# utiasDSL/safe-control-gym

Hardware: AMD Instinct MI355X
Metric: env-steps/sec (whole node), Quadrotor2D-track (higher is better)
Workload: dtype f32; 1 GPU; quadrotor_2D_track: 65536 envs/GPU x 1 GPU, 1 launch of the fused step kernel per control step (20 engine substeps, obs/reward/done/info/constraints, auto-reset), synthetic U(-1,1) actions resident in HBM, HIP graph of 82 steps; envs_per_gpu=65536, task_yaml=safe_control_gym_amd/configs/quadrotor_2D_track.yaml, parallelism=env-shard x1, rccl_ranks=1, kernel_build=config-specialised, timing=one timed region of 82 steps

## Files before the change

### include/scg_learn.h

```cpp
#ifndef SCG_LEARN_H
#define SCG_LEARN_H

#include <stddef.h>
#include <stdint.h>

#ifdef __cplusplus
extern "C" {
#endif

typedef struct {
    int32_t W1, b1;
    int32_t W2, b2;
    int32_t W3, b3;
} scg_mlp_layout;

void scg_learn_shape(int32_t* obs_dim, int32_t* hidden, int32_t* act_dim, int32_t* activation);

int scg_mlp_forward(const float* d_params, const scg_mlp_layout* layout, int nout, const float* d_x, int m, float* d_out,
                    const uint8_t* d_row_mask, void* stream);

typedef struct {
    const float* d_params;
    scg_mlp_layout actor, critic;
    int32_t logstd_off;
    int32_t n_params;
    const float* d_obs;
    const float* d_act;
    const float* d_logp_old;
    const float* d_adv;
    const float* d_ret;
    const float* d_v_old;
    const int32_t* d_idx;
    int32_t batch;
    float clip_param, entropy_coef;
    int32_t use_clipped_value;
    int32_t n_workgroups;
    void* d_workspace;
    float* d_grad;
    float* d_stats;
} scg_ppo_grad_args;
size_t scg_ppo_grad_workspace_bytes(int n_workgroups);
int scg_ppo_grad(const scg_ppo_grad_args* args, void* stream);

int scg_adam_gated(float* d_p, const float* d_g, float* d_m, float* d_v, int n, int n_actor, float lr_actor, float lr_critic,
                   float* d_steps, float target_kl, float* d_stats_acc, const float* d_stats, uint32_t* d_block_counter,
                   void* stream);
int scg_adam_gated_scaled(float* d_p, const float* d_g, float* d_m, float* d_v, int n, int n_actor, float lr_actor, float lr_critic,
                          float* d_steps, float target_kl, float* d_stats_acc, const float* d_stats, uint32_t* d_block_counter,
                          float grad_scale, void* stream);

int scg_ppo_step(const scg_ppo_grad_args* args, float* d_m, float* d_v, float lr_actor, float lr_critic, const float* d_steps_in,
                 float* d_steps_out, float target_kl, float* d_stats_acc, void* stream);

void scg_learn_force_accumulating_form(int on);

int scg_ppo_returns_prepare(const uint8_t* d_done, const uint8_t* d_flags, const float* d_rew, const float* d_v_all, int T, int N,
                            uint8_t* d_trunc, float* d_mask, float* d_rew_out, float* d_v_out, void* stream);
size_t scg_ppo_returns_scratch_bytes(void);
int scg_ppo_returns_moments(const float* d_adv, int T, int N, float* d_episode_acc, void* d_scratch, double* d_moments,
                            float* d_episode_totals, void* stream);
int scg_ppo_returns_normalise(const float* d_adv, const double* d_moments, int T, int N, float* d_out, void* stream);

int scg_random_permutation(int32_t* d_out, int n, int count, uint64_t key, void* stream);
int scg_random_permutation_keyed(int32_t* d_out, int n, int count, const uint64_t* d_key_state, uint32_t epoch_offset, void* stream);

const char* scg_learn_last_error(void);
const char* scg_learn_source_hash_tag(void);

#ifdef __cplusplus
}
#endif
#endif
```

### safe_control_gym_amd/_learn.py

```python
import ctypes as C
import os

from safe_control_gym_amd import _lib as L
from safe_control_gym_amd import _shapelib

ACTS = {'tanh': 0, 'relu': 1, 'leaky_relu': 2}
SRC = os.path.join(L.CSRC_DIR, 'scg_learn.hip')
DEPS = [SRC, os.path.join(L.CSRC_DIR, 'scg_adam.h'), os.path.join(L.CSRC_DIR, 'scg_mlp.h'), os.path.join(L.CSRC_DIR, 'scg_once.h'), os.path.normpath(os.path.join(L.CSRC_DIR, '..', '..', 'include', 'scg_learn.h'))]


class MlpLayout(C.Structure):
    _fields_ = [(n, C.c_int32) for n in ('W1', 'b1', 'W2', 'b2', 'W3', 'b3')]


class PpoGradArgs(C.Structure):
    _fields_ = [('d_params', C.c_void_p), ('actor', MlpLayout), ('critic', MlpLayout), ('logstd_off', C.c_int32),
                ('n_params', C.c_int32), ('d_obs', C.c_void_p), ('d_act', C.c_void_p), ('d_logp_old', C.c_void_p),
                ('d_adv', C.c_void_p), ('d_ret', C.c_void_p), ('d_v_old', C.c_void_p), ('d_idx', C.c_void_p),
                ('batch', C.c_int32), ('clip_param', C.c_float), ('entropy_coef', C.c_float),
                ('use_clipped_value', C.c_int32), ('n_workgroups', C.c_int32), ('d_workspace', C.c_void_p),
                ('d_grad', C.c_void_p), ('d_stats', C.c_void_p)]


def supported(obs_dim, hidden, act_dim, activation):
    return (1 <= obs_dim <= 31 and hidden % 32 == 0 and 32 <= hidden <= 128 and act_dim in (1, 2, 4) and activation in ACTS)


def source_hash():
    return _shapelib.source_hash(DEPS)


def lib_path(obs_dim, hidden, act_dim, activation):
    tag = os.environ.get('SCG_LEARN_TAG', '')
    return os.path.join(L.SPEC_DIR, f'libscg_learn_{obs_dim}_{hidden}_{act_dim}_{activation}{"_" + tag if tag else ""}.so')


def build(obs_dim, hidden, act_dim, activation, force=False):
    if not supported(obs_dim, hidden, act_dim, activation):
        raise L.ScgError(f'no MFMA learner for obs {obs_dim} hidden {hidden} act {act_dim} {activation}')
    defines = {'SCG_L_NIN': obs_dim, 'SCG_L_H': hidden, 'SCG_L_NU': act_dim, 'SCG_L_ACT': ACTS[activation]}
    return _shapelib.build(lib_path(obs_dim, hidden, act_dim, activation), SRC, DEPS, defines, 'learner', 'SCG_LEARN_FLAGS', force)
# ... 36 lines not shown
```

### safe_control_gym_amd/csrc/scg_learn.hip

```cpp
#include <hip/hip_runtime.h>

#include <algorithm>
#include <cstdint>
#include <cstdio>
#include <cstdlib>
#include <string>

#include "../../include/scg_learn.h"
#include "scg_adam.h"
#include "scg_mlp.h"
#include "scg_once.h"

#ifndef SCG_L_NIN
#error "compile with -DSCG_L_NIN= -DSCG_L_H= -DSCG_L_NU= -DSCG_L_ACT="
#endif

using namespace scg;

#ifndef SCG_L_PART_AUX
#define SCG_L_PART_AUX 17
#endif
constexpr int NIN = SCG_L_NIN, HID = SCG_L_H, NU = SCG_L_NU, ACT = SCG_L_ACT;
constexpr int NT = HID / 32;
constexpr int XS_WORDS = (NIN + 2) * 32;
constexpr int WAVES = 4;

static thread_local std::string g_err;
static int fail(int code, const std::string& m) { g_err = m; return code; }
extern "C" const char* scg_learn_last_error(void) { return g_err.c_str(); }
extern "C" void scg_learn_shape(int32_t* nin, int32_t* hidden, int32_t* nu, int32_t* act) {
    *nin = NIN; *hidden = HID; *nu = NU; *act = ACT;
}
#ifndef SCG_SRC_HASH
#define SCG_SRC_HASH 0ULL
#endif
#define SCG_STR2(x) #x
#define SCG_STR(x) SCG_STR2(x)
extern "C" const char* scg_learn_source_hash_tag(void) { return "SCG_SRC_HASH:" SCG_STR(SCG_SRC_HASH); }

#define HIP_TRY(e) do { hipError_t _e = (e); if (_e != hipSuccess) return fail(-2, std::string(#e) + ": " + hipGetErrorString(_e)); } while (0)

__host__ __device__ static inline MlpWeights weights_of(const float* p, const scg_mlp_layout& L) {
    return MlpWeights{p + L.W1, p + L.b1, p + L.W2, p + L.b2, p + L.W3, p + L.b3};
}

template <int L1Q>
__device__ __forceinline__ void load_x(const float* __restrict__ obs, int sample, int h, float* x) {
#pragma unroll
    for (int g = 0; g < L1Q / 4; ++g) {
        const int r0 = 8 * g + 4 * h;
        if constexpr (NIN % 4 == 0) {
            f32x4 v = {0.0f, 0.0f, 0.0f, 0.0f};
            if (r0 < NIN) v = *reinterpret_cast<const f32x4*>(obs + (size_t)sample * NIN + r0);
            x[4 * g + 0] = v.x; x[4 * g + 1] = v.y; x[4 * g + 2] = v.z; x[4 * g + 3] = v.w;
        } else {
#pragma unroll
            for (int r = 0; r < 4; ++r) x[4 * g + r] = (r0 + r < NIN) ? obs[(size_t)sample * NIN + r0 + r] : 0.0f;
        }
    }
}

#ifndef SCG_L_FWD_WAVES
#define SCG_L_FWD_WAVES 8
#endif
constexpr int FWD_WAVES = SCG_L_FWD_WAVES;
constexpr int FWD_FILL = FWD_WAVES > 8 ? 512 : 64 * FWD_WAVES;
template <int NOUT>
__global__ __launch_bounds__(64 * FWD_WAVES) void mlp_forward_kernel(const float* __restrict__ params, const scg_mlp_layout lay,
                                                          const float* __restrict__ xin, int M, float* __restrict__ out,
                                                          const uint8_t* __restrict__ row_mask) {
    using L = MlpLds<NIN, HID, NOUT>;
    extern __shared__ __align__(16) float lds[];
    const MlpWeights w = weights_of(params, lay);
    if (FWD_FILL == 64 * FWD_WAVES || (int)threadIdx.x < FWD_FILL) mlp_fill_lds<NIN, HID, NOUT, 20, FWD_FILL>(lds, w, threadIdx.x);
    __syncthreads();
    const int lane = threadIdx.x & 63, wave = threadIdx.x >> 6;
    const int c = lane & 31, h = lane >> 5;
    const int n_tiles = (M + 31) / 32;
    for (int tile = blockIdx.x * (blockDim.x >> 6) + wave; tile < n_tiles; tile += gridDim.x * (blockDim.x >> 6)) {
        int s = tile * 32 + c;
        const bool live = s < M;
        s = live ? s : M - 1;
        if (row_mask) {
            const bool want = live && row_mask[s] != 0;
            if (__ballot(want) == 0ull) {
                if (live && h == 0) {
#pragma unroll
                    for (int k = 0; k < NOUT; ++k) out[(size_t)s * NOUT + k] = 0.0f;
                }
                continue;
            }
        }
        float x[L::L1Q];
        load_x<L::L1Q>(xin, s, h, x);
        f32x16 h1[NT], h2[NT];
        float o[NOUT];
        mlp_forward_tile<NIN, HID, NOUT, ACT>(lds, x, h1, h2, o, lane);
        if (live && h == 0) {
            const bool keep = !row_mask || row_mask[s] != 0;
#pragma unroll
            for (int k = 0; k < NOUT; ++k) out[(size_t)s * NOUT + k] = keep ? o[k] : 0.0f;
        }
    }
}

template <int NOUT>
struct GradLds {
    static constexpr int DW1 = 0;
    static constexpr int DB1 = DW1 + NIN * HID;
    static constexpr int DB2 = DB1 + HID;
    static constexpr int DW3 = DB2 + HID;
    static constexpr int DB3 = DW3 + NOUT * HID;
    static constexpr int DLS = DB3 + 4;
    static constexpr int STAT = DLS + 4;
    static constexpr int END = STAT + 4;
};
template <int NOUT> constexpr int partial_small() { return GradLds<NOUT>::END; }
template <int NOUT> constexpr int partial_words() { return GradLds<NOUT>::END + HID * HID; }
constexpr int PARTIAL_STRIDE = partial_words<(NU > 1 ? NU : 1)>();

constexpr int W1R = GradLds<(NU > 1 ? NU : 1)>::END;
constexpr size_t grad_lds_base_words() {
    size_t a = MlpLds<NIN, HID, NU>::END + GradLds<NU>::END;
    size_t c = MlpLds<NIN, HID, 1>::END + GradLds<1>::END;
    return (a > c ? a : c) + WAVES * XS_WORDS + WAVES * 4 * 32 + WAVES * TR_WORDS;
}
constexpr bool private_dw1() { return (grad_lds_base_words() + (WAVES - 1) * W1R) * sizeof(float) <= 160 * 1024; }
constexpr int PUB_TILE = 1024;
constexpr size_t scratch_words() { return WAVES * XS_WORDS + WAVES * 4 * 32 + WAVES * TR_WORDS + (private_dw1() ? (WAVES - 1) * W1R : 0); }
template <int NOUT>
constexpr size_t region_b_words() {
    constexpr size_t in_image = MlpLds<NIN, HID, NOUT>::END / PUB_TILE, need = 2 * WAVES * (HID / 32);
    constexpr size_t rest = need > in_image ? (need - in_image) * PUB_TILE : 0;
    return rest > scratch_words() ? rest : scratch_words();
}
static_assert(NIN < 32, "the dW1 product appends a column of ones: NIN + 1 <= 32");

struct GradArgs {
    const float* params; scg_mlp_layout actor, critic; int logstd_off;
    const float* obs; const float* act; const float* logp_old; const float* adv; const float* ret; const float* v_old;
    const int32_t* idx; int batch;
    float clip_param; int use_clipped_value;
    float* partials;
};

#ifdef SCG_L_TIMING
#define SCG_L_SLOTS reinterpret_cast<unsigned long long*>(A.partials + (size_t)gridDim.x * 2 * PARTIAL_STRIDE)
#define SCG_L_STAMP(k) do { if (ACTOR && blockIdx.x == 0 && threadIdx.x == 0) SCG_L_SLOTS[k] = __builtin_readcyclecounter(); } while (0)
#define SCG_L_TSTAMP(k) do { tst[k] = __builtin_readcyclecounter(); } while (0)
#else
#define SCG_L_STAMP(k) do {} while (0)
#define SCG_L_TSTAMP(k) do {} while (0)
#endif

__device__ __forceinline__ void gl_add(float* p, float v) {
    if constexpr (private_dw1()) *p += v;
    else atomicAdd(p, v);
}

template <int NOUT, bool ACTOR, bool ONE>
__device__ __forceinline__ void grad_net(const GradArgs& A, float* lds) {
    using L = MlpLds<NIN, HID, NOUT>;
    using G = GradLds<NOUT>;
    constexpr int L1Q = L::L1Q;
    float* const gl = lds + L::END;
    float* const xs_all = gl + G::END;
    float* const dout_all = xs_all + WAVES * XS_WORDS;
    float* const scr_all = dout_all + WAVES * 4 * 32;
    float* const w1_all = scr_all + WAVES * TR_WORDS;
    const int tid = threadIdx.x, lane = tid & 63, wave = tid >> 6;
    const int c = lane & 31, h = lane >> 5;
    const MlpWeights w = weights_of(A.params, ACTOR ? A.actor : A.critic);
    SCG_L_STAMP(0);
    const int n_tiles = A.batch / 32;
    const int tile0 = blockIdx.x * WAVES + wave;
    const int s_pre = A.idx[tile0 < n_tiles ? tile0 * 32 + c : c];
    float x_pre[L1Q], act_pre[NOUT], a_pre = 0.0f, b_pre = 0.0f;
    if constexpr (ONE) {
        mlp_fill_lds<NIN, HID, NOUT>(lds, w, tid, [&]() {
            load_x<L1Q>(A.obs, s_pre, h, x_pre);
            if constexpr (ACTOR) {
#pragma unroll
                for (int a = 0; a < NOUT; ++a) act_pre[a] = A.act[(size_t)s_pre * NOUT + a];
                a_pre = A.logp_old[s_pre]; b_pre = A.adv[s_pre];
            } else {
                a_pre = A.ret[s_pre];
                if (A.use_clipped_value) b_pre = A.v_old[s_pre];
            }
        });
    } else {
        mlp_fill_lds<NIN, HID, NOUT>(lds, w, tid);
    }
    for (int k = tid; k < G::END; k += blockDim.x) gl[k] = 0.0f;
    if constexpr (private_dw1()) {
// ... 37 lines not shown
#ifdef SCG_L_TIMING
        unsigned long long tst[10];
#endif
        SCG_L_TSTAMP(0);
        float x[L1Q];
        float s_act[NOUT], s_a = 0.0f, s_b = 0.0f;
        if constexpr (ONE) {
#pragma unroll
            for (int q = 0; q < L1Q; ++q) x[q] = x_pre[q];
#pragma unroll
            for (int a = 0; a < NOUT; ++a) s_act[a] = act_pre[a];
            s_a = a_pre; s_b = b_pre;
        } else {
            const int s = tile == tile0 ? s_pre : A.idx[tile * 32 + c];
            load_x<L1Q>(A.obs, s, h, x);
            if constexpr (ACTOR) {
#pragma unroll
                for (int a = 0; a < NOUT; ++a) s_act[a] = A.act[(size_t)s * NOUT + a];
                s_a = A.logp_old[s]; s_b = A.adv[s];
            } else {
                s_a = A.ret[s];
                if (A.use_clipped_value) s_b = A.v_old[s];
            }
        }
#pragma unroll
        for (int q = 0; q < L1Q; ++q) {
            const int f = d_row(q, 0);
            if (f + 4 < NIN) xs[(f + 4 * h) * 32 + c] = x[q];
            else if (f < NIN) { if (h == 0) xs[f * 32 + c] = x[q]; }
        }
        SCG_L_TSTAMP(1);
        float out[NOUT], dout[NOUT];
#ifdef SCG_L_TIMING
        mlp_forward_tile<NIN, HID, NOUT, ACT, 20, ACT, ONE>(lds, x, h1, h2, out, lane, tst + 8);
#else
        mlp_forward_tile<NIN, HID, NOUT, ACT, 20, ACT, ONE>(lds, x, h1, h2, out, lane);
#endif
        SCG_L_TSTAMP(2);
        if constexpr (ACTOR) {
            float logp = 0.0f, z[NOUT];
#pragma unroll
            for (int a = 0; a < NOUT; ++a) {
                z[a] = (s_act[a] - out[a]) * inv_std[a];
                logp += -0.5f * z[a] * z[a] - logstd[a] - 0.91893853320467274f;
            }
            const float lp_old = s_a, adv = s_b;
            const float ratio = __expf(logp - lp_old);
            const float lo = 1.0f - A.clip_param, hi = 1.0f + A.clip_param;
            const float rc = fminf(fmaxf(ratio, lo), hi);
            const float s1 = ratio * adv, s2 = rc * adv;
            const bool inside = ratio >= lo && ratio <= hi;
            const float dsur = (inside || s1 < s2) ? adv : 0.0f;
            const float wl = -dsur * ratio * inv_b;
#pragma unroll
            for (int a = 0; a < NOUT; ++a) {
                dout[a] = wl * z[a] * inv_std[a];
                if (h == 0) dls[a] += wl * (z[a] * z[a] - 1.0f);
            }
            if (h == 0) { st_loss += -fminf(s1, s2) * inv_b; st_kl += (lp_old - logp) * inv_b; }
        } else {
            const float v = out[0], ret = s_a;
            float dv = v - ret, l = dv * dv;
            if (A.use_clipped_value) {
                const float vo = s_b;
                const float d = v - vo;
                const float vc = vo + fminf(fmaxf(d, -A.clip_param), A.clip_param);
                const float e2 = vc - ret, l2 = e2 * e2;
                const float pass = (d >= -A.clip_param && d <= A.clip_param) ? 1.0f : 0.0f;
                if (l2 > l) { dv = e2 * pass; l = l2; }
                else if (l2 == l) dv = 0.5f * (dv + e2 * pass);
            }
            dout[0] = dv * inv_b;
            if (h == 0) st_loss += 0.5f * l * inv_b;
        }
        if (h == 0) {
#pragma unroll
            for (int o = 0; o < NOUT; ++o) dout_l[o * 32 + c] = dout[o];
        }
        __builtin_amdgcn_fence(__ATOMIC_RELEASE, "wavefront");
        __builtin_amdgcn_wave_barrier();
        __builtin_amdgcn_fence(__ATOMIC_ACQUIRE, "wavefront");
        if (lane < NOUT) {
            float v = 0.0f;
#pragma unroll
            for (int g = 0; g < 8; ++g) {
                const f32x4 d4 = *reinterpret_cast<const f32x4*>(dout_l + lane * 32 + 4 * g);
                v += d4.x; v += d4.y; v += d4.z; v += d4.w;
            }
            gl_add(glw + G::DB3 + lane, v);
        }
        SCG_L_TSTAMP(3);
#ifndef DBG_NO_DW3
#pragma unroll
        for (int tau = 0; tau < NT; ++tau) {
            float t[16];
            tile_transpose(scr, h2[tau], t, lane);
            float a3[NOUT], x3[NOUT];
#pragma unroll
            for (int o = 0; o < NOUT; ++o) {
                float acc = 0.0f;
#pragma unroll
                for (int g = 0; g < 4; ++g) {
                    const f32x4 dv = *reinterpret_cast<const f32x4*>(dout_l + o * 32 + 8 * g + 4 * h);
                    acc = __builtin_fmaf(t[4 * g], dv.x, acc); acc = __builtin_fmaf(t[4 * g + 1], dv.y, acc);
                    acc = __builtin_fmaf(t[4 * g + 2], dv.z, acc); acc = __builtin_fmaf(t[4 * g + 3], dv.w, acc);
                }
                a3[o] = acc;
            }
#pragma unroll
            for (int o = 0; o < NOUT; ++o) x3[o] = __shfl_xor(a3[o], 32, 64);
            if (h == 0) {
#pragma unroll
                for (int o = 0; o < NOUT; ++o) gl_add(glw + G::DW3 + o * HID + 32 * tau + c, a3[o] + x3[o]);
            }
        }
#endif
        SCG_L_TSTAMP(4);
#pragma unroll
        for (int tau = 0; tau < NT; ++tau) {
#pragma unroll
            for (int g = 0; g < 4; ++g) {
                float dh[4] = {0.0f, 0.0f, 0.0f, 0.0f};
#pragma unroll
                for (int o = 0; o < NOUT; ++o) {
                    const f32x4 wv = *reinterpret_cast<const f32x4*>(lds + L::W3 + o * HID + 32 * tau + 8 * g + 4 * h);
                    dh[0] = __builtin_fmaf(wv.x, dout[o], dh[0]); dh[1] = __builtin_fmaf(wv.y, dout[o], dh[1]);
                    dh[2] = __builtin_fmaf(wv.z, dout[o], dh[2]); dh[3] = __builtin_fmaf(wv.w, dout[o], dh[3]);
                }
#pragma unroll
                for (int r = 0; r < 4; ++r) h2[tau][4 * g + r] = dh[r] * mlp_dact<ACT>(h2[tau][4 * g + r]);
            }
        }
#pragma unroll
        for (int tau = 0; tau < NT; ++tau) tile_transpose_inplace(scr, h1[tau], lane);
        SCG_L_TSTAMP(5);
        __builtin_amdgcn_sched_barrier(0);
        {
            const int ip = lane & 31;
            const int qi = 4 * (ip >> 3) + (ip & 3), hi2 = (ip >> 2) & 1;
            const float* const xrow = xs + (c < NIN + 1 ? c : NIN + 1) * 32 + 4 * h;
            float a_nx[16];
            auto gather = [&](int tp, int rp, float* a) {
                const float* base = lds + L::W2F + (rp * NT + tp) * L::TILE2 + 32 * hi2 * L::S + qi;
#pragma unroll
                for (int q = 0; q < 16; ++q) a[q] = base[d_row(q, h) * L::S];
            };
            if constexpr (ONE) gather(0, 0, a_nx);
#pragma unroll
            for (int tp = 0; tp < NT; ++tp) {
                f32x16 acc;
#pragma unroll
                for (int q = 0; q < 16; ++q) acc[q] = 0.0f;
#pragma unroll
                for (int rp = 0; rp < NT; ++rp) {
                    float a[16];
                    if constexpr (ONE) {
#pragma unroll
                        for (int q = 0; q < 16; ++q) a[q] = a_nx[q];
                        if (rp + 1 < NT) gather(tp, rp + 1, a_nx);
                        else if (tp + 1 < NT) gather(tp + 1, 0, a_nx);
                    } else {
                        gather(tp, rp, a);
                    }
#pragma unroll
                    for (int q = 0; q < 16; ++q) acc = mfma32(h2[rp][q], a[q], acc);
                    __builtin_amdgcn_sched_barrier(0);
                }
#pragma unroll
                for (int q = 0; q < 16; ++q) acc[q] *= mlp_dact<ACT>(h1[tp][q]);
#ifndef DBG_NO_DW1
// ... 200 lines not shown
                if (tau != ((wave + r) % WAVES)) continue;
#pragma unroll
                for (int rho = 0; rho < NT; ++rho) {
                    float* const p = stg + ((tau * NT + rho) * 4 * 64 + lane) * 4;
#pragma unroll
                    for (int g = 0; g < 4; ++g) {
                        f32x4 v = {dW2[tau][rho][4 * g], dW2[tau][rho][4 * g + 1], dW2[tau][rho][4 * g + 2], dW2[tau][rho][4 * g + 3]};
                        if (r > 0) v += *reinterpret_cast<const f32x4*>(p + 256 * g);
                        *reinterpret_cast<f32x4*>(p + 256 * g) = v;
                    }
                }
            }
            __syncthreads();
        }
    }
    SCG_L_STAMP(4);
    for (int k = 4 * tid; k < G::END; k += 4 * blockDim.x)
        __builtin_amdgcn_raw_buffer_store_b128(__builtin_bit_cast(u32x4, *reinterpret_cast<const f32x4*>(gl + k)), pr, pbase + 4u * (uint32_t)k, 0, SCG_L_PART_AUX);
    if constexpr (!ONE) {
        for (int k = 4 * tid; k < HID * HID; k += 4 * blockDim.x)
            __builtin_amdgcn_raw_buffer_store_b128(__builtin_bit_cast(u32x4, *reinterpret_cast<const f32x4*>(stg + k)), pr, pbase + 4u * (uint32_t)(G::END + k), 0,
                                                   SCG_L_PART_AUX);
    }
    SCG_L_STAMP(5);
}

constexpr size_t grad_lds_words() {
    size_t a = MlpLds<NIN, HID, NU>::END + GradLds<NU>::END + region_b_words<NU>();
    size_t c = MlpLds<NIN, HID, 1>::END + GradLds<1>::END + region_b_words<1>();
    return a > c ? a : c;
}
static_assert(grad_lds_words() * sizeof(float) <= 160 * 1024, "the gradient kernel's LDS does not fit");

template <bool ONE>
__global__ __launch_bounds__(64 * WAVES, 1) void ppo_grad_kernel(const GradArgs A) {
    extern __shared__ __align__(16) float lds[];
    if (blockIdx.y == 0) grad_net<NU, true, ONE>(A, lds);
    else grad_net<1, false, ONE>(A, lds);
}
static int g_force_accumulating = getenv("SCG_LEARN_MULTI_TILE") != nullptr;
extern "C" void scg_learn_force_accumulating_form(int on) { g_force_accumulating = on != 0; }
static int launch_grad(const GradArgs& G, int n_workgroups, hipStream_t st) {
    const size_t bytes = grad_lds_words() * sizeof(float);
    static scg::PerDeviceOnce set_g;
    int dev;
    if (set_g.pending(&dev)) {
        HIP_TRY(hipFuncSetAttribute((const void*)ppo_grad_kernel<false>, hipFuncAttributeMaxDynamicSharedMemorySize, (int)bytes));
        HIP_TRY(hipFuncSetAttribute((const void*)ppo_grad_kernel<true>, hipFuncAttributeMaxDynamicSharedMemorySize, (int)bytes));
        set_g.commit(dev);
    }
    if (G.batch / 32 <= n_workgroups * WAVES && !g_force_accumulating) ppo_grad_kernel<true><<<dim3(n_workgroups, 2), dim3(64 * WAVES), bytes, st>>>(G);
    else ppo_grad_kernel<false><<<dim3(n_workgroups, 2), dim3(64 * WAVES), bytes, st>>>(G);
    HIP_TRY(hipGetLastError());
    return 0;
}

struct ReduceArgs {
    const float* partials; int n_wg;
    scg_mlp_layout actor, critic; int logstd_off; int n_params;
    float entropy_coef;
    const float* params;
    float* grad;
    float* stats;
};

template <int NOUT>
__device__ __forceinline__ int dest_of(int k, const scg_mlp_layout& lay, int logstd_off, bool actor) {
    using G = GradLds<NOUT>;
    if (k < G::DB1) { const int in = k / HID, o = k % HID; return lay.W1 + o * NIN + in; }
    if (k < G::DB2) return lay.b1 + (k - G::DB1);
    if (k < G::DW3) return lay.b2 + (k - G::DB2);
    if (k < G::DB3) return lay.W3 + (k - G::DW3);
    if (k < G::DLS) return (k - G::DB3) < NOUT ? lay.b3 + (k - G::DB3) : -1;
    if (k < G::STAT) return (actor && (k - G::DLS) < NOUT) ? logstd_off + (k - G::DLS) : -1;
    if (k < G::END) return -2 - (k - G::STAT);
    const int p = k - G::END;
    const int q = 4 * ((p >> 8) & 3) + (p & 3), lane = (p >> 2) & 63, tr = p >> 10;
    const int tau = tr / NT, rho = tr % NT;
    return lay.W2 + (32 * rho + (lane & 31)) * HID + 32 * tau + d_row(q, lane >> 5);
}

__global__ __launch_bounds__(256) void ppo_reduce_kernel(const ReduceArgs R) {
    __shared__ float part[4][64];
    const int net = blockIdx.y;
    const int kl = threadIdx.x & 63, grp = threadIdx.x >> 6;
// ... 292 lines not shown
    while (bits < 31 && (1u << bits) < (uint32_t)n) ++bits;
    const int half = (bits + 1) / 2;
    permutation_kernel<false><<<dim3((count + 255) / 256), dim3(256), 0, (hipStream_t)stream>>>(
        d_out, (uint32_t)n, (uint32_t)count, half, (uint32_t)key, (uint32_t)(key >> 32), nullptr, 0u);
    HIP_TRY(hipGetLastError());
    return 0;
}
extern "C" int scg_random_permutation_keyed(int32_t* d_out, int n, int count, const uint64_t* d_key_state, uint32_t epoch_offset, void* stream) {
    if (!d_out || !d_key_state || n <= 0 || count < 0 || count > n) return fail(-1, "scg_random_permutation_keyed: bad argument");
    if (count == 0) return 0;
    int bits = 1;
    while (bits < 31 && (1u << bits) < (uint32_t)n) ++bits;
    const int half = (bits + 1) / 2;
    permutation_kernel<true><<<dim3((count + 255) / 256), dim3(256), 0, (hipStream_t)stream>>>(
        d_out, (uint32_t)n, (uint32_t)count, half, 0u, 0u, d_key_state, epoch_offset);
    HIP_TRY(hipGetLastError());
    return 0;
}
extern "C" int scg_mlp_forward(const float* d_params, const scg_mlp_layout* layout, int nout, const float* d_x, int m,
                               float* d_out, const uint8_t* d_row_mask, void* stream) {
    if (!d_params || !layout || !d_x || !d_out || m <= 0) return fail(-1, "scg_mlp_forward: bad argument");
    static int n_cu = 0;
    if (!n_cu) {
        int dev = 0, v = 0;
        if (hipGetDevice(&dev) == hipSuccess && hipDeviceGetAttribute(&v, hipDeviceAttributeMultiprocessorCount, dev) == hipSuccess && v > 2) n_cu = v;
        else n_cu = 256;
    }
    const int grid = std::min(std::max(n_cu - 2, 1), (m + 32 * FWD_WAVES - 1) / (32 * FWD_WAVES));
    hipStream_t st = (hipStream_t)stream;
    if (nout == NU) {
        const size_t bytes = MlpLds<NIN, HID, NU>::END * sizeof(float);
        static scg::PerDeviceOnce set_a;
        int dev;
        if (set_a.pending(&dev)) { HIP_TRY(hipFuncSetAttribute((const void*)mlp_forward_kernel<NU>, hipFuncAttributeMaxDynamicSharedMemorySize, (int)bytes)); set_a.commit(dev); }
        mlp_forward_kernel<NU><<<dim3(grid), dim3(64 * FWD_WAVES), bytes, st>>>(d_params, *layout, d_x, m, d_out, d_row_mask);
    } else if (nout == 1) {
        const size_t bytes = MlpLds<NIN, HID, 1>::END * sizeof(float);
        static scg::PerDeviceOnce set_c;
        int dev;
        if (set_c.pending(&dev)) { HIP_TRY(hipFuncSetAttribute((const void*)mlp_forward_kernel<1>, hipFuncAttributeMaxDynamicSharedMemorySize, (int)bytes)); set_c.commit(dev); }
        mlp_forward_kernel<1><<<dim3(grid), dim3(64 * FWD_WAVES), bytes, st>>>(d_params, *layout, d_x, m, d_out, d_row_mask);
    } else {
        return fail(-1, "scg_mlp_forward: this library serves nout = act_dim or 1");
    }
    HIP_TRY(hipGetLastError());
    return 0;
}

extern "C" size_t scg_ppo_grad_workspace_bytes(int n_workgroups) {
    size_t b = (size_t)n_workgroups * 2 * PARTIAL_STRIDE * sizeof(float);
#ifdef SCG_L_TIMING
    b += 256;
#endif
    return b;
}

extern "C" int scg_ppo_grad(const scg_ppo_grad_args* a, void* stream) {
    if (!a || !a->d_params || !a->d_obs || !a->d_act || !a->d_logp_old || !a->d_adv || !a->d_ret || !a->d_v_old || !a->d_idx ||
        !a->d_workspace || !a->d_grad || !a->d_stats)
        return fail(-1, "scg_ppo_grad: NULL argument");
    if (a->batch <= 0 || a->batch % 32 != 0) return fail(-1, "scg_ppo_grad: the minibatch size must be a positive multiple of 32");
    if (a->n_workgroups <= 0) return fail(-1, "scg_ppo_grad: n_workgroups must be positive");
    hipStream_t st = (hipStream_t)stream;
    GradArgs G;
    G.params = a->d_params; G.actor = a->actor; G.critic = a->critic; G.logstd_off = a->logstd_off;
    G.obs = a->d_obs; G.act = a->d_act; G.logp_old = a->d_logp_old; G.adv = a->d_adv; G.ret = a->d_ret; G.v_old = a->d_v_old;
    G.idx = a->d_idx; G.batch = a->batch; G.clip_param = a->clip_param; G.use_clipped_value = a->use_clipped_value;
    G.partials = (float*)a->d_workspace;
    if (int rc = launch_grad(G, a->n_workgroups, st)) return rc;
    ReduceArgs R;
    R.partials = G.partials; R.n_wg = a->n_workgroups; R.actor = a->actor; R.critic = a->critic; R.logstd_off = a->logstd_off;
    R.n_params = a->n_params; R.entropy_coef = a->entropy_coef; R.params = a->d_params; R.grad = a->d_grad; R.stats = a->d_stats;
    ppo_reduce_kernel<<<dim3((PARTIAL_STRIDE + 63) / 64, 2), dim3(256), 0, st>>>(R);
    HIP_TRY(hipGetLastError());
// ... 44 lines not shown
```

Baseline: 15.29 billion env-steps/s.

## Overlap activation and transpose work under MFMA in learner MLP forward/backward

Adds overlapped variants of the MLP forward tile and the one-tile PPO gradient backward pass. Activations, dz2 products, dW3 reductions and tile transposes are interleaved with the MFMA chains using sched_group_barrier hints and prefetched W2 gathers. The goal is to hide VALU and LDS latency behind matrix instructions. A serial fallback stays available through a force flag, at the cost of more code variants and greater register pressure.

```diff
diff --git a/include/scg_learn.h b/include/scg_learn.h
--- a/include/scg_learn.h
+++ b/include/scg_learn.h
@@ -54,6 +54,8 @@
 
 void scg_learn_force_accumulating_form(int on);
 
+void scg_learn_force_serial_tiles(int on);
+
 int scg_ppo_returns_prepare(const uint8_t* d_done, const uint8_t* d_flags, const float* d_rew, const float* d_v_all, int T, int N,
                             uint8_t* d_trunc, float* d_mask, float* d_rew_out, float* d_v_out, void* stream);
 size_t scg_ppo_returns_scratch_bytes(void);
diff --git a/safe_control_gym_amd/_learn.py b/safe_control_gym_amd/_learn.py
--- a/safe_control_gym_amd/_learn.py
+++ b/safe_control_gym_amd/_learn.py
@@ -6,7 +6,7 @@
 
 ACTS = {'tanh': 0, 'relu': 1, 'leaky_relu': 2}
 SRC = os.path.join(L.CSRC_DIR, 'scg_learn.hip')
-DEPS = [SRC, os.path.join(L.CSRC_DIR, 'scg_adam.h'), os.path.join(L.CSRC_DIR, 'scg_mlp.h'), os.path.join(L.CSRC_DIR, 'scg_once.h'), os.path.normpath(os.path.join(L.CSRC_DIR, '..', '..', 'include', 'scg_learn.h'))]
+DEPS = [SRC, os.path.join(L.CSRC_DIR, 'scg_adam.h'), os.path.join(L.CSRC_DIR, 'scg_mlp.h'), os.path.join(L.CSRC_DIR, 'scg_mlp_overlap.h'), os.path.join(L.CSRC_DIR, 'scg_once.h'), os.path.normpath(os.path.join(L.CSRC_DIR, '..', '..', 'include', 'scg_learn.h'))]
 
 
 class MlpLayout(C.Structure):
diff --git a/safe_control_gym_amd/csrc/scg_learn.hip b/safe_control_gym_amd/csrc/scg_learn.hip
--- a/safe_control_gym_amd/csrc/scg_learn.hip
+++ b/safe_control_gym_amd/csrc/scg_learn.hip
@@ -9,6 +9,7 @@
 #include "../../include/scg_learn.h"
 #include "scg_adam.h"
 #include "scg_mlp.h"
+#include "scg_mlp_overlap.h"
 #include "scg_once.h"
 
 #ifndef SCG_L_NIN
@@ -65,7 +66,7 @@
 #endif
 constexpr int FWD_WAVES = SCG_L_FWD_WAVES;
 constexpr int FWD_FILL = FWD_WAVES > 8 ? 512 : 64 * FWD_WAVES;
-template <int NOUT>
+template <int NOUT, bool OVL>
 __global__ __launch_bounds__(64 * FWD_WAVES) void mlp_forward_kernel(const float* __restrict__ params, const scg_mlp_layout lay,
                                                           const float* __restrict__ xin, int M, float* __restrict__ out,
                                                           const uint8_t* __restrict__ row_mask) {
@@ -95,7 +96,8 @@
         load_x<L::L1Q>(xin, s, h, x);
         f32x16 h1[NT], h2[NT];
         float o[NOUT];
-        mlp_forward_tile<NIN, HID, NOUT, ACT>(lds, x, h1, h2, o, lane);
+        if constexpr (OVL) mlp_forward_tile_overlap<NIN, HID, NOUT, ACT>(lds, x, h1, h2, o, lane);
+        else mlp_forward_tile<NIN, HID, NOUT, ACT>(lds, x, h1, h2, o, lane);
         if (live && h == 0) {
             const bool keep = !row_mask || row_mask[s] != 0;
 #pragma unroll
@@ -158,8 +160,12 @@
     else atomicAdd(p, v);
 }
 
-template <int NOUT, bool ACTOR, bool ONE>
+#ifndef SCG_L_OVL_BWD
+#define SCG_L_OVL_BWD 1
+#endif
+template <int NOUT, bool ACTOR, bool ONE, bool OVL>
 __device__ __forceinline__ void grad_net(const GradArgs& A, float* lds) {
+    constexpr bool OVLB = OVL && SCG_L_OVL_BWD != 0;
     using L = MlpLds<NIN, HID, NOUT>;
     using G = GradLds<NOUT>;
     constexpr int L1Q = L::L1Q;
@@ -263,10 +269,12 @@
         SCG_L_TSTAMP(1);
         float out[NOUT], dout[NOUT];
 #ifdef SCG_L_TIMING
-        mlp_forward_tile<NIN, HID, NOUT, ACT, 20, ACT, ONE>(lds, x, h1, h2, out, lane, tst + 8);
+        unsigned long long* const fts = tst + 8;
 #else
-        mlp_forward_tile<NIN, HID, NOUT, ACT, 20, ACT, ONE>(lds, x, h1, h2, out, lane);
-#endif
+        unsigned long long* const fts = nullptr;
+#endif
+        if constexpr (OVL) mlp_forward_tile_overlap<NIN, HID, NOUT, ACT, 20, ACT, ONE>(lds, x, h1, h2, out, lane, fts);
+        else mlp_forward_tile<NIN, HID, NOUT, ACT, 20, ACT, ONE>(lds, x, h1, h2, out, lane, fts);
         SCG_L_TSTAMP(2);
         if constexpr (ACTOR) {
             float logp = 0.0f, z[NOUT];
@@ -321,9 +329,7 @@
             gl_add(glw + G::DB3 + lane, v);
         }
         SCG_L_TSTAMP(3);
-#ifndef DBG_NO_DW3
-#pragma unroll
-        for (int tau = 0; tau < NT; ++tau) {
+        auto dw3_products = [&](int tau, float* a3s) {
             float t[16];
             tile_transpose(scr, h2[tau], t, lane);
             float a3[NOUT], x3[NOUT];
@@ -340,15 +346,16 @@
             }
 #pragma unroll
             for (int o = 0; o < NOUT; ++o) x3[o] = __shfl_xor(a3[o], 32, 64);
+#pragma unroll
+            for (int o = 0; o < NOUT; ++o) a3s[o] = a3[o] + x3[o];
+        };
+        auto dw3_add = [&](int tau, const float* a3s) {
             if (h == 0) {
 #pragma unroll
-                for (int o = 0; o < NOUT; ++o) gl_add(glw + G::DW3 + o * HID + 32 * tau + c, a3[o] + x3[o]);
-            }
-        }
-#endif
-        SCG_L_TSTAMP(4);
-#pragma unroll
-        for (int tau = 0; tau < NT; ++tau) {
+                for (int o = 0; o < NOUT; ++o) gl_add(glw + G::DW3 + o * HID + 32 * tau + c, a3s[o]);
+            }
+        };
+        auto dz2_tile = [&](int tau) {
 #pragma unroll
             for (int g = 0; g < 4; ++g) {
                 float dh[4] = {0.0f, 0.0f, 0.0f, 0.0f};
@@ -361,12 +368,240 @@
 #pragma unroll
                 for (int r = 0; r < 4; ++r) h2[tau][4 * g + r] = dh[r] * mlp_dact<ACT>(h2[tau][4 * g + r]);
             }
-        }
-#pragma unroll
-        for (int tau = 0; tau < NT; ++tau) tile_transpose_inplace(scr, h1[tau], lane);
-        SCG_L_TSTAMP(5);
-        __builtin_amdgcn_sched_barrier(0);
-        {
+        };
+        if constexpr (!OVLB) {
+#ifndef DBG_NO_DW3
+#pragma unroll
+            for (int tau = 0; tau < NT; ++tau) {
+                float t[16];
+                tile_transpose(scr, h2[tau], t, lane);
+                float a3[NOUT], x3[NOUT];
+#pragma unroll
+                for (int o = 0; o < NOUT; ++o) {
+                    float acc = 0.0f;
+#pragma unroll
+                    for (int g = 0; g < 4; ++g) {
+                        const f32x4 dv = *reinterpret_cast<const f32x4*>(dout_l + o * 32 + 8 * g + 4 * h);
+                        acc = __builtin_fmaf(t[4 * g], dv.x, acc); acc = __builtin_fmaf(t[4 * g + 1], dv.y, acc);
+                        acc = __builtin_fmaf(t[4 * g + 2], dv.z, acc); acc = __builtin_fmaf(t[4 * g + 3], dv.w, acc);
+                    }
+                    a3[o] = acc;
+                }
+#pragma unroll
+                for (int o = 0; o < NOUT; ++o) x3[o] = __shfl_xor(a3[o], 32, 64);
+                if (h == 0) {
+#pragma unroll
+                    for (int o = 0; o < NOUT; ++o) gl_add(glw + G::DW3 + o * HID + 32 * tau + c, a3[o] + x3[o]);
+                }
+            }
+#endif
+            SCG_L_TSTAMP(4);
+#pragma unroll
+            for (int tau = 0; tau < NT; ++tau) {
+#pragma unroll
+                for (int g = 0; g < 4; ++g) {
+                    float dh[4] = {0.0f, 0.0f, 0.0f, 0.0f};
+#pragma unroll
+                    for (int o = 0; o < NOUT; ++o) {
+                        const f32x4 wv = *reinterpret_cast<const f32x4*>(lds + L::W3 + o * HID + 32 * tau + 8 * g + 4 * h);
+                        dh[0] = __builtin_fmaf(wv.x, dout[o], dh[0]); dh[1] = __builtin_fmaf(wv.y, dout[o], dh[1]);
+                        dh[2] = __builtin_fmaf(wv.z, dout[o], dh[2]); dh[3] = __builtin_fmaf(wv.w, dout[o], dh[3]);
+                    }
+#pragma unroll
+                    for (int r = 0; r < 4; ++r) h2[tau][4 * g + r] = dh[r] * mlp_dact<ACT>(h2[tau][4 * g + r]);
+                }
+            }
+#pragma unroll
+            for (int tau = 0; tau < NT; ++tau) tile_transpose_inplace(scr, h1[tau], lane);
+            SCG_L_TSTAMP(5);
+            __builtin_amdgcn_sched_barrier(0);
+        }
+        if constexpr (OVLB) {
+            static_assert(ONE, "the overlapped tile is the one-tile form's (the accumulating form has no registers for it)");
+            constexpr int SG_FILL = SG_VALU | SG_TRANS | 0x80;
+            constexpr int N_DZ2 = 20 * NOUT + 16 * (1 + ActCost<ACT>::DACT_OPS), N_TR = 24;
+            float a3s[NOUT];
+#ifndef DBG_NO_DW3
+            dw3_products(0, a3s);
+            dw3_add(0, a3s);
+#endif
+            SCG_L_TSTAMP(4);
+            dz2_tile(0);
+            SCG_L_TSTAMP(5);
+            __builtin_amdgcn_sched_barrier(0);
+            const int ip = lane & 31;
+            const int qi = 4 * (ip >> 3) + (ip & 3), hi2 = (ip >> 2) & 1;
+            const float* const xrow = xs + (c < NIN + 1 ? c : NIN + 1) * 32 + 4 * h;
+            auto gather = [&](int tp, int rp, float* a) {
+                const float* base = lds + L::W2F + (rp * NT + tp) * L::TILE2 + 32 * hi2 * L::S + qi;
+#pragma unroll
+                for (int q = 0; q < 16; ++q) a[q] = base[d_row(q, h) * L::S];
+            };
+            auto tr_write = [&](const f32x16& tile) {
+                float* const wr = scr + 4 * h * TR_STRIDE + c;
+#pragma unroll
+                for (int q = 0; q < 16; ++q) wr[d_row(q, 0) * TR_STRIDE] = tile[q];
+            };
+            auto wave_sync = [&]() {
+                __builtin_amdgcn_fence(__ATOMIC_RELEASE, "wavefront");
+                __builtin_amdgcn_wave_barrier();
+                __builtin_amdgcn_fence(__ATOMIC_ACQUIRE, "wavefront");
+            };
+            auto tr_read = [&](float* t) {
+                const float* const rd = scr + c * TR_STRIDE + 4 * h;
+#pragma unroll
+                for (int g = 0; g < 4; ++g) {
+                    const f32x4 v = *reinterpret_cast<const f32x4*>(rd + 8 * g);
+                    t[4 * g] = v.x; t[4 * g + 1] = v.y; t[4 * g + 2] = v.z; t[4 * g + 3] = v.w;
+                }
+            };
+            float a_nx[16];
+            gather(0, 0, a_nx);
+            f32x16 acc[NT];
+#pragma unroll
+            for (int tp = 0; tp < NT; ++tp)
+#pragma unroll
+                for (int q = 0; q < 16; ++q) acc[tp][q] = 0.0f;
+#pragma unroll
+            for (int rp = 0; rp < NT; ++rp) {
+#pragma unroll
+                for (int tp = 0; tp < NT; ++tp) {
+                    float a[16];
+#pragma unroll
+                    for (int q = 0; q < 16; ++q) a[q] = a_nx[q];
+                    if (tp + 1 < NT) gather(tp + 1, rp, a_nx);
+                    else if (rp + 1 < NT) gather(0, rp + 1, a_nx);
+                    constexpr int TR_AT = NT >= 3 ? 2 : 1;
+#ifndef DBG_NO_DW3
+                    if (rp + 1 < NT && tp == 0) {
+                        float t[16];
+                        f32x4 dv[NOUT][4];
+#pragma unroll
+                        for (int q = 0; q < 4; ++q) acc[tp] = mfma32(h2[rp][q], a[q], acc[tp]);
+                        tr_write(h2[rp + 1]);
+#pragma unroll
+                        for (int i = 0; i < 4; ++i) { __builtin_amdgcn_sched_group_barrier(SG_MFMA, 1, 0); __builtin_amdgcn_sched_group_barrier(SG_DS_WRITE, 4, 0); }
+                        __builtin_amdgcn_sched_barrier(0);
+                        wave_sync();
+#pragma unroll
+                        for (int q = 4; q < 8; ++q) acc[tp] = mfma32(h2[rp][q], a[q], acc[tp]);
+                        tr_read(t);
+#pragma unroll
+                        for (int o = 0; o < NOUT; ++o)
+#pragma unroll
+                            for (int g = 0; g < 4; ++g) dv[o][g] = *reinterpret_cast<const f32x4*>(dout_l + o * 32 + 8 * g + 4 * h);
+#pragma unroll
+                        for (int i = 0; i < 4; ++i) { __builtin_amdgcn_sched_group_barrier(SG_MFMA, 1, 0); __builtin_amdgcn_sched_group_barrier(SG_DS_READ, 1 + NOUT, 0); }
+                        __builtin_amdgcn_sched_barrier(0);
+                        wave_sync();
+#pragma unroll
+                        for (int q = 8; q < 16; ++q) acc[tp] = mfma32(h2[rp][q], a[q], acc[tp]);
+                        float a3[NOUT], x3[NOUT];
+#pragma unroll
+                        for (int o = 0; o < NOUT; ++o) {
+                            float s3 = 0.0f;
+#pragma unroll
+                            for (int g = 0; g < 4; ++g) {
+                                s3 = __builtin_fmaf(t[4 * g], dv[o][g].x, s3); s3 = __builtin_fmaf(t[4 * g + 1], dv[o][g].y, s3);
+                                s3 = __builtin_fmaf(t[4 * g + 2], dv[o][g].z, s3); s3 = __builtin_fmaf(t[4 * g + 3], dv[o][g].w, s3);
+                            }
+                            a3[o] = s3;
+                        }
+#pragma unroll
+                        for (int o = 0; o < NOUT; ++o) x3[o] = __shfl_xor(a3[o], 32, 64);
+#pragma unroll
+                        for (int o = 0; o < NOUT; ++o) a3s[o] = a3[o] + x3[o];
+#pragma unroll
+                        for (int i = 0; i < 8; ++i) { __builtin_amdgcn_sched_group_barrier(SG_MFMA, 1, 0); __builtin_amdgcn_sched_group_barrier(SG_VALU, 2 * NOUT + 1, 0); }
+                        __builtin_amdgcn_sched_barrier(0);
+                        dw3_add(rp + 1, a3s);
+                        continue;
+                    }
+#endif
+#pragma unroll
+                    for (int q = 0; q < 16; ++q) acc[tp] = mfma32(h2[rp][q], a[q], acc[tp]);
+                    if (rp + 1 < NT) {
+                        if (tp == 1) {
+                            dz2_tile(rp + 1);
+                            if (TR_AT == 1) tile_transpose_inplace(scr, h1[rp], lane);
+                            sched_fill_under_mfma<15, (N_DZ2 + (TR_AT == 1 ? N_TR : 0) + 14) / 15 + 1, 1, (TR_AT == 1 ? SG_FILL : SG_VALU | SG_TRANS)>();
+                        } else if (tp == TR_AT) {
+                            tile_transpose_inplace(scr, h1[rp], lane);
+                            sched_fill_under_mfma<15, (N_TR + 14) / 15 + 1, 1, SG_FILL>();
+                        }
+                    } else if (tp == 0) {
+                        tile_transpose_inplace(scr, h1[rp], lane);
+                        sched_fill_under_mfma<15, (N_TR + 14) / 15 + 1, 1, SG_FILL>();
+                    }
+                    __builtin_amdgcn_sched_barrier(0);
+                }
+            }
+            float* const dst0 = w1 + (c <= NIN ? c : NIN) * HID + 4 * h;
+            auto g1_load = [&](int tp, f32x16& g1) {
+                if constexpr (private_dw1()) {
+#pragma unroll
+                    for (int g = 0; g < 4; ++g) {
+                        const f32x4 v = *reinterpret_cast<const f32x4*>(dst0 + 32 * tp + 8 * g);
+                        g1[4 * g] = v.x; g1[4 * g + 1] = v.y; g1[4 * g + 2] = v.z; g1[4 * g + 3] = v.w;
+                    }
+                } else {
+#pragma unroll
+                    for (int q = 0; q < 16; ++q) g1[q] = 0.0f;
+                }
+            };
+            auto g1_store = [&](int tp, const f32x16& g1) {
+                if (c <= NIN) {
+                    if constexpr (private_dw1()) {
+#pragma unroll
+                        for (int g = 0; g < 4; ++g)
+                            *reinterpret_cast<f32x4*>(dst0 + 32 * tp + 8 * g) = (f32x4){g1[4 * g], g1[4 * g + 1], g1[4 * g + 2], g1[4 * g + 3]};
+                    } else {
+#pragma unroll
+                        for (int q = 0; q < 16; ++q) atomicAdd(dst0 + 32 * tp + d_row(q, 0), g1[q]);
+                    }
+                }
+            };
+#pragma unroll
+            for (int q = 0; q < 16; ++q) acc[0][q] *= mlp_dact<ACT>(h1[0][q]);
+#ifndef DBG_NO_DW1
+            float xb[16];
+#pragma unroll
+            for (int g = 0; g < 4; ++g) {
+                const f32x4 v = *reinterpret_cast<const f32x4*>(xrow + 8 * g);
+                xb[4 * g] = v.x; xb[4 * g + 1] = v.y; xb[4 * g + 2] = v.z; xb[4 * g + 3] = v.w;
+            }
+            f32x16 g1[NT];
+            g1_load(0, g1[0]);
+#endif
+            __builtin_amdgcn_sched_barrier(0);
+#pragma unroll
+            for (int tp = 0; tp < NT; ++tp) {
+#ifndef DBG_NO_DW1
+                if (tp + 1 < NT) g1_load(tp + 1, g1[tp + 1]);
+#endif
+#pragma unroll
+                for (int q = 0; q < 16; ++q) {
+#ifndef DBG_NO_DW1
+                    g1[tp] = mfma32(acc[tp][q], xb[q], g1[tp]);
+#endif
+                    if (tp + 1 < NT) {
+                        float y = acc[tp + 1][q];
+                        pin_here(y);
+                        y *= mlp_dact<ACT>(h1[tp + 1][q]);
+                        pin_here(y);
+                        acc[tp + 1][q] = y;
+                    }
+                    __builtin_amdgcn_sched_barrier(0);
+                }
+#ifndef DBG_NO_DW1
+                if (tp > 0) g1_store(tp - 1, g1[tp - 1]);
+#endif
+            }
+#ifndef DBG_NO_DW1
+            g1_store(NT - 1, g1[NT - 1]);
+#endif
+            __builtin_amdgcn_sched_barrier(0);
+        } else {
             const int ip = lane & 31;
             const int qi = 4 * (ip >> 3) + (ip & 3), hi2 = (ip >> 2) & 1;
             const float* const xrow = xs + (c < NIN + 1 ? c : NIN + 1) * 32 + 4 * h;
@@ -633,25 +868,31 @@
 }
 static_assert(grad_lds_words() * sizeof(float) <= 160 * 1024, "the gradient kernel's LDS does not fit");
 
-template <bool ONE>
+template <bool ONE, bool OVL>
 __global__ __launch_bounds__(64 * WAVES, 1) void ppo_grad_kernel(const GradArgs A) {
     extern __shared__ __align__(16) float lds[];
-    if (blockIdx.y == 0) grad_net<NU, true, ONE>(A, lds);
-    else grad_net<1, false, ONE>(A, lds);
+    if (blockIdx.y == 0) grad_net<NU, true, ONE, OVL>(A, lds);
+    else grad_net<1, false, ONE, OVL>(A, lds);
 }
 static int g_force_accumulating = getenv("SCG_LEARN_MULTI_TILE") != nullptr;
 extern "C" void scg_learn_force_accumulating_form(int on) { g_force_accumulating = on != 0; }
+static int g_force_serial = 0;
+extern "C" void scg_learn_force_serial_tiles(int on) { g_force_serial = on != 0; }
 static int launch_grad(const GradArgs& G, int n_workgroups, hipStream_t st) {
     const size_t bytes = grad_lds_words() * sizeof(float);
     static scg::PerDeviceOnce set_g;
     int dev;
     if (set_g.pending(&dev)) {
-        HIP_TRY(hipFuncSetAttribute((const void*)ppo_grad_kernel<false>, hipFuncAttributeMaxDynamicSharedMemorySize, (int)bytes));
-        HIP_TRY(hipFuncSetAttribute((const void*)ppo_grad_kernel<true>, hipFuncAttributeMaxDynamicSharedMemorySize, (int)bytes));
+        HIP_TRY(hipFuncSetAttribute((const void*)ppo_grad_kernel<false, false>, hipFuncAttributeMaxDynamicSharedMemorySize, (int)bytes));
+        HIP_TRY(hipFuncSetAttribute((const void*)ppo_grad_kernel<true, false>, hipFuncAttributeMaxDynamicSharedMemorySize, (int)bytes));
+        HIP_TRY(hipFuncSetAttribute((const void*)ppo_grad_kernel<true, true>, hipFuncAttributeMaxDynamicSharedMemorySize, (int)bytes));
         set_g.commit(dev);
     }
-    if (G.batch / 32 <= n_workgroups * WAVES && !g_force_accumulating) ppo_grad_kernel<true><<<dim3(n_workgroups, 2), dim3(64 * WAVES), bytes, st>>>(G);
-    else ppo_grad_kernel<false><<<dim3(n_workgroups, 2), dim3(64 * WAVES), bytes, st>>>(G);
+    const dim3 grid(n_workgroups, 2), block(64 * WAVES);
+    const bool one = G.batch / 32 <= n_workgroups * WAVES && !g_force_accumulating;
+    if (one && !g_force_serial) ppo_grad_kernel<true, true><<<grid, block, bytes, st>>>(G);
+    else if (one) ppo_grad_kernel<true, false><<<grid, block, bytes, st>>>(G);
+    else ppo_grad_kernel<false, false><<<grid, block, bytes, st>>>(G);
     HIP_TRY(hipGetLastError());
     return 0;
 }
@@ -1010,14 +1251,24 @@
         const size_t bytes = MlpLds<NIN, HID, NU>::END * sizeof(float);
         static scg::PerDeviceOnce set_a;
         int dev;
-        if (set_a.pending(&dev)) { HIP_TRY(hipFuncSetAttribute((const void*)mlp_forward_kernel<NU>, hipFuncAttributeMaxDynamicSharedMemorySize, (int)bytes)); set_a.commit(dev); }
-        mlp_forward_kernel<NU><<<dim3(grid), dim3(64 * FWD_WAVES), bytes, st>>>(d_params, *layout, d_x, m, d_out, d_row_mask);
+        if (set_a.pending(&dev)) {
+            HIP_TRY(hipFuncSetAttribute((const void*)mlp_forward_kernel<NU, true>, hipFuncAttributeMaxDynamicSharedMemorySize, (int)bytes));
+            HIP_TRY(hipFuncSetAttribute((const void*)mlp_forward_kernel<NU, false>, hipFuncAttributeMaxDynamicSharedMemorySize, (int)bytes));
+            set_a.commit(dev);
+        }
+        if (!g_force_serial) mlp_forward_kernel<NU, true><<<dim3(grid), dim3(64 * FWD_WAVES), bytes, st>>>(d_params, *layout, d_x, m, d_out, d_row_mask);
+        else mlp_forward_kernel<NU, false><<<dim3(grid), dim3(64 * FWD_WAVES), bytes, st>>>(d_params, *layout, d_x, m, d_out, d_row_mask);
     } else if (nout == 1) {
         const size_t bytes = MlpLds<NIN, HID, 1>::END * sizeof(float);
         static scg::PerDeviceOnce set_c;
         int dev;
-        if (set_c.pending(&dev)) { HIP_TRY(hipFuncSetAttribute((const void*)mlp_forward_kernel<1>, hipFuncAttributeMaxDynamicSharedMemorySize, (int)bytes)); set_c.commit(dev); }
-        mlp_forward_kernel<1><<<dim3(grid), dim3(64 * FWD_WAVES), bytes, st>>>(d_params, *layout, d_x, m, d_out, d_row_mask);
+        if (set_c.pending(&dev)) {
+            HIP_TRY(hipFuncSetAttribute((const void*)mlp_forward_kernel<1, true>, hipFuncAttributeMaxDynamicSharedMemorySize, (int)bytes));
+            HIP_TRY(hipFuncSetAttribute((const void*)mlp_forward_kernel<1, false>, hipFuncAttributeMaxDynamicSharedMemorySize, (int)bytes));
+            set_c.commit(dev);
+        }
+        if (!g_force_serial) mlp_forward_kernel<1, true><<<dim3(grid), dim3(64 * FWD_WAVES), bytes, st>>>(d_params, *layout, d_x, m, d_out, d_row_mask);
+        else mlp_forward_kernel<1, false><<<dim3(grid), dim3(64 * FWD_WAVES), bytes, st>>>(d_params, *layout, d_x, m, d_out, d_row_mask);
     } else {
         return fail(-1, "scg_mlp_forward: this library serves nout = act_dim or 1");
     }
diff --git a/safe_control_gym_amd/csrc/scg_mlp_overlap.h b/safe_control_gym_amd/csrc/scg_mlp_overlap.h
--- /dev/null
+++ b/safe_control_gym_amd/csrc/scg_mlp_overlap.h
@@ -0,0 +1,114 @@
+#pragma once
+#include "scg_mlp.h"
+
+namespace scg {
+
+enum { SG_VALU = 0x2, SG_MFMA = 0x8, SG_DS_READ = 0x100, SG_DS_WRITE = 0x200, SG_TRANS = 0x400 };
+
+template <int ACT> struct ActCost { static constexpr int ACT_OPS = 3, DACT_OPS = 3; };
+template <> struct ActCost<MLP_ACT_TANH> { static constexpr int ACT_OPS = 5, DACT_OPS = 2; };
+template <> struct ActCost<MLP_ACT_RELU> { static constexpr int ACT_OPS = 1, DACT_OPS = 3; };
+template <> struct ActCost<MLP_ACT_NONE> { static constexpr int ACT_OPS = 0, DACT_OPS = 0; };
+
+template <int N, int OPS, int LEAD = 1, int MASK = SG_VALU | SG_TRANS>
+__device__ __forceinline__ void sched_fill_under_mfma() {
+    if constexpr (OPS > 0) {
+        __builtin_amdgcn_sched_group_barrier(SG_MFMA, LEAD, 0);
+#pragma unroll
+        for (int i = 0; i < N; ++i) {
+            __builtin_amdgcn_sched_group_barrier(MASK, OPS, 0);
+            __builtin_amdgcn_sched_group_barrier(SG_MFMA, 1, 0);
+        }
+    }
+}
+
+__device__ __forceinline__ void pin_here(float& v) { asm volatile("" : "+v"(v)); }
+
+template <int NIN, int H, int NOUT, int ACT, int SS = 20, int ACT2 = ACT, bool PF = false>
+__device__ __forceinline__ void mlp_forward_tile_overlap(const float* lds, const float* x, f32x16* h1, f32x16* h2, float* out, int lane,
+                                                         unsigned long long* ts = nullptr) {
+    using L = MlpLds<NIN, H, NOUT, SS>;
+    constexpr int NT = L::NT, L1Q = L::L1Q;
+    const int h = lane >> 5;
+#pragma unroll
+    for (int rho = 0; rho < NT; ++rho) {
+        f32x16 acc;
+#pragma unroll
+        for (int g = 0; g < 4; ++g) {
+            const f32x4 b = *reinterpret_cast<const f32x4*>(lds + L::B1 + 32 * rho + 8 * g + 4 * h);
+            acc[4 * g + 0] = b.x; acc[4 * g + 1] = b.y; acc[4 * g + 2] = b.z; acc[4 * g + 3] = b.w;
+        }
+#pragma unroll
+        for (int q = 0; q < L1Q; ++q) acc = mfma32(lds[L::W1F + (rho * L1Q + q) * 64 + lane], x[q], acc);
+        if (rho > 0) {
+#pragma unroll
+            for (int q = 0; q < 16; ++q) h1[rho - 1][q] = mlp_act<ACT>(h1[rho - 1][q]);
+            sched_fill_under_mfma<L1Q - 1, (16 + L1Q - 2) / (L1Q - 1) * ActCost<ACT>::ACT_OPS>();
+        }
+        __builtin_amdgcn_sched_barrier(0);
+        h1[rho] = acc;
+    }
+    if constexpr (NT == 1) {
+#pragma unroll
+        for (int q = 0; q < 16; ++q) h1[0][q] = mlp_act<ACT>(h1[0][q]);
+    }
+    if (ts) ts[0] = __builtin_readcyclecounter();
+    float a_nx[16];
+    if constexpr (PF) load_w2_tile<L>(lds, 0, 0, lane, a_nx);
+#pragma unroll
+    for (int rho = 0; rho < NT; ++rho) {
+        f32x16 acc;
+#pragma unroll
+        for (int g = 0; g < 4; ++g) {
+            const f32x4 b = *reinterpret_cast<const f32x4*>(lds + L::B2 + 32 * rho + 8 * g + 4 * h);
+            acc[4 * g + 0] = b.x; acc[4 * g + 1] = b.y; acc[4 * g + 2] = b.z; acc[4 * g + 3] = b.w;
+        }
+#pragma unroll
+        for (int tau = 0; tau < NT; ++tau) {
+            float a[16];
+            if constexpr (PF) {
+#pragma unroll
+                for (int q = 0; q < 16; ++q) a[q] = a_nx[q];
+                if (tau + 1 < NT) load_w2_tile<L>(lds, rho, tau + 1, lane, a_nx);
+                else if (rho + 1 < NT) load_w2_tile<L>(lds, rho + 1, 0, lane, a_nx);
+            } else {
+                load_w2_tile<L>(lds, rho, tau, lane, a);
+            }
+#pragma unroll
+            for (int q = 0; q < 16; ++q) acc = mfma32(a[q], h1[tau][q], acc);
+            if (tau == 0 && NT > 1) {
+                if (rho == 0) {
+#pragma unroll
+                    for (int q = 0; q < 16; ++q) h1[NT - 1][q] = mlp_act<ACT>(h1[NT - 1][q]);
+                    sched_fill_under_mfma<15, ActCost<ACT>::ACT_OPS>();
+                } else {
+#pragma unroll
+                    for (int q = 0; q < 16; ++q) h2[rho - 1][q] = mlp_act<ACT2>(h2[rho - 1][q]);
+                    sched_fill_under_mfma<15, ActCost<ACT2>::ACT_OPS>();
+                }
+            }
+            __builtin_amdgcn_sched_barrier(0);
+        }
+        h2[rho] = acc;
+    }
+#pragma unroll
+    for (int q = 0; q < 16; ++q) h2[NT - 1][q] = mlp_act<ACT2>(h2[NT - 1][q]);
+    if (ts) ts[1] = __builtin_readcyclecounter();
+#pragma unroll
+    for (int o = 0; o < NOUT; ++o) {
+        float s = 0.0f;
+#pragma unroll
+        for (int tau = 0; tau < NT; ++tau) {
+#pragma unroll
+            for (int g = 0; g < 4; ++g) {
+                const f32x4 w = *reinterpret_cast<const f32x4*>(lds + L::W3 + o * H + 32 * tau + 8 * g + 4 * h);
+                s = __builtin_fmaf(w.x, h2[tau][4 * g + 0], s); s = __builtin_fmaf(w.y, h2[tau][4 * g + 1], s);
+                s = __builtin_fmaf(w.z, h2[tau][4 * g + 2], s); s = __builtin_fmaf(w.w, h2[tau][4 * g + 3], s);
+            }
+        }
+        s += __shfl_xor(s, 32, 64);
+        out[o] = s + lds[L::B3 + o];
+    }
+}
+
+}
```

Measured after the change: 15.33 billion env-steps/s, median of 3. Within noise of the previous version (+0.3%).
